# ziadabohalawa/6DoF-Pose-Estimation-and-Defect-Projection

Measured on AMD Instinct MI355X. Metric: Mrays/s ray-mesh + ICP iters/s, 640x576 vs 100k-tri mesh, higher is better.
Workload: dtype f32 rays / f64 ICP (f32 MFMA filter)

## Files before the change

6dof-pose-estimation-and-defect-projection_amd/_lib.py:

```python
import ctypes as C
import os
import sys
import threading

import numpy as np

_HERE = os.path.dirname(os.path.abspath(__file__))
LIB_PATH = os.environ.get("PEDP_LIB", os.path.join(_HERE, "libpedp_hip.so"))

HOST, DEVICE = 0, 1
POINT_TO_PLANE, POINT_TO_POINT = 0, 1


class PreprocessParams(C.Structure):
    _fields_ = [("voxel_size", C.c_double), ("plane_distance", C.c_double), ("plane_iterations", C.c_int32),
                ("first_frame", C.c_int32), ("seed", C.c_uint64), ("normal_radius", C.c_double), ("normal_max_nn", C.c_int32),
                ("cluster_min_points", C.c_int32), ("cluster_eps", C.c_double), ("outlier_neighbors", C.c_int32),
                ("flags", C.c_int32), ("outlier_std_ratio", C.c_double), ("average_normal_voxel", C.c_double)]

ALLREDUCE_FN = C.CFUNCTYPE(C.c_int, C.c_void_p, C.c_void_p, C.c_int, C.c_void_p)


class IcpParams(C.Structure):
    _fields_ = [
# ... 71 lines not shown
    "pedp_cloud_create": (C.c_int, [C.c_void_p, C.c_void_p, C.c_void_p, C.c_int64, _P(C.c_void_p)]),
    "pedp_cloud_create_device": (C.c_int, [C.c_void_p, C.c_void_p, C.c_void_p, C.c_int64, _P(C.c_void_p)]),
    "pedp_cloud_destroy": (None, [C.c_void_p]),
    "pedp_cloud_size": (C.c_int, [C.c_void_p, _P(C.c_int64), _P(C.c_int)]),
    "pedp_icp_graph_captures": (C.c_int, [C.c_void_p, _P(C.c_int64)]),
    "pedp_cloud_set_target_order": (C.c_int, [C.c_void_p, C.c_int]),
    "pedp_cloud_target_order": (C.c_int, [C.c_void_p, _P(C.c_int)]),
    "pedp_debug_target_pack": (C.c_int, [C.c_void_p, C.c_void_p, _P(C.c_int64), _P(C.c_int64), C.c_void_p, C.c_void_p,
                                         C.c_void_p, C.c_void_p, C.c_void_p]),
    "pedp_icp": (C.c_int, [C.c_void_p, C.c_void_p, C.c_void_p, _P(IcpParams), C.c_void_p, C.c_void_p,
                           _P(C.c_double), _P(C.c_double), _P(C.c_int32), C.c_void_p, C.c_void_p]),
    "pedp_icp_batched": (C.c_int, [C.c_void_p, C.c_void_p, C.c_void_p, _P(IcpParams), C.c_void_p, C.c_int,
                                   C.c_void_p, C.c_void_p, C.c_void_p]),
    "pedp_icp_batched_ex": (C.c_int, [C.c_void_p, C.c_void_p, C.c_void_p, _P(IcpParams), C.c_void_p, C.c_int,
                                      C.c_void_p, C.c_void_p, C.c_void_p, C.c_void_p]),
    "pedp_nn": (C.c_int, [C.c_void_p, C.c_void_p, C.c_void_p, C.c_void_p, C.c_void_p, C.c_void_p]),
    "pedp_nn_last_sweep_ms": (C.c_int, [C.c_void_p, _P(C.c_float)]),
    "pedp_icp_last_stats": (C.c_int, [C.c_void_p, _P(C.c_int64), _P(C.c_int64), _P(C.c_int64)]),
    "pedp_icp_last_planned_passes": (C.c_int, [C.c_void_p, _P(C.c_int64)]),
    "pedp_icp_last_serial_path": (C.c_int, [C.c_void_p, _P(C.c_int64), _P(C.c_int64)]),
    "pedp_icp_last_head_closed": (C.c_int, [C.c_void_p, _P(C.c_int64), _P(C.c_int64), _P(C.c_int64)]),
    "pedp_icp_last_certified": (C.c_int, [C.c_void_p, _P(C.c_int64), _P(C.c_int64)]),
    "pedp_icp_last_steady": (C.c_int, [C.c_void_p, _P(C.c_int64), _P(C.c_int64)]),
    "pedp_debug_nn_bf16": (C.c_int, [C.c_void_p, C.c_void_p, C.c_int64, C.c_void_p, C.c_int64, C.c_void_p]),
    "pedp_debug_icp_path": (C.c_int, [C.c_void_p, C.c_void_p, C.c_void_p]),
    "pedp_icp_begin": (C.c_int, [C.c_void_p, C.c_void_p, C.c_void_p, _P(IcpParams), C.c_void_p, C.c_int]),
    "pedp_icp_end": (C.c_int, [C.c_void_p, C.c_void_p, _P(C.c_double), _P(C.c_double), _P(C.c_int32), C.c_void_p, C.c_void_p]),
    "pedp_icp_configure": (C.c_int, [C.c_void_p, C.c_int, C.c_int]),
    "pedp_comm_unique_id": (C.c_int, [C.c_void_p]),
    "pedp_comm_create": (C.c_int, [C.c_void_p, C.c_void_p, C.c_int, C.c_int]),
    "pedp_comm_destroy": (C.c_int, [C.c_void_p]),
    "pedp_comm_size": (C.c_int, [C.c_void_p, _P(C.c_int), _P(C.c_int)]),
    "pedp_comm_allgather": (C.c_int, [C.c_void_p, C.c_void_p, C.c_void_p, C.c_int64]),
    "pedp_comm_allreduce_f64": (C.c_int, [C.c_void_p, C.c_void_p, C.c_int64]),
    "pedp_render": (C.c_int, [C.c_void_p, C.c_void_p, C.c_int64, C.c_void_p, C.c_int64, C.c_void_p, C.c_void_p, C.c_void_p,
                              C.c_void_p, C.c_int, C.c_int, C.c_void_p, C.c_void_p, C.c_int, C.c_void_p, C.c_int, C.c_void_p,
                              C.c_void_p, C.c_void_p, C.c_void_p]),
    "pedp_rasterize": (C.c_int, [C.c_void_p, C.c_void_p, C.c_int, C.c_int64, C.c_void_p, C.c_int64, C.c_int, C.c_int, C.c_int,
                                 C.c_void_p]),
    "pedp_interpolate": (C.c_int, [C.c_void_p, C.c_void_p, C.c_int, C.c_int64, C.c_int, C.c_void_p, C.c_int, C.c_int, C.c_int,
                                   C.c_void_p, C.c_int64, C.c_int, C.c_void_p]),
    "pedp_texture": (C.c_int, [C.c_void_p, C.c_void_p, C.c_int, C.c_int, C.c_int, C.c_int, C.c_void_p, C.c_int, C.c_int, C.c_int,
                               C.c_int, C.c_void_p]),
    "pedp_render_configure": (C.c_int, [C.c_void_p, C.c_int]),
    "pedp_warp_perspective": (C.c_int, [C.c_void_p, C.c_void_p, C.c_void_p, C.c_int, C.c_int, C.c_int, C.c_int, C.c_int,
                                        C.c_int, C.c_void_p]),
# ... 629 lines not shown
    a, b = C.c_int64(0), C.c_int64(0)
    check(load().pedp_icp_last_serial_path(ctx._h, C.byref(a), C.byref(b)), "pedp_icp_last_serial_path")
    return a.value, b.value


def icp_last_head_closed(ctx, rebuilds=False):
    a, b, c = C.c_int64(0), C.c_int64(0), C.c_int64(0)
    check(load().pedp_icp_last_head_closed(ctx._h, C.byref(a), C.byref(b), C.byref(c)), "pedp_icp_last_head_closed")
    return (a.value, b.value, c.value) if rebuilds else a.value


def icp_last_certified(ctx):
    a, b = C.c_int64(0), C.c_int64(0)
    check(load().pedp_icp_last_certified(ctx._h, C.byref(a), C.byref(b)), "pedp_icp_last_certified")
    return a.value, b.value


def icp_last_steady(ctx):
    a, b = C.c_int64(0), C.c_int64(0)
    check(load().pedp_icp_last_steady(ctx._h, C.byref(a), C.byref(b)), "pedp_icp_last_steady")
    return a.value, b.value


ICP_SWITCHES = ("nn_f32", "unfused_finish", "no_visit_plan", "serial_close", "copy_bracket", "head_close", "cert", "steady")
ICP_PATH_FIELDS = ("fused", "dev_result", "copy_bracket", "head", "certify", "plan", "serial_close", "unfused_finish", "exchange",
                   "steady", "steady_from")


class IcpSwitches(C.Structure):
    _fields_ = [(n, C.c_int) for n in ICP_SWITCHES + ("steady_from", "steady_grid", "target_order")]


class IcpPathInputs(C.Structure):
    _fields_ = [("n_source", C.c_int64), ("n_target", C.c_int64), ("radius", C.c_double)] + [
        (n, C.c_int) for n in ("unit_size", "poses", "timed_pass", "exhaustive", "exchange", "batch", "early_exit", "no_steady", "resident")]


class IcpPath(C.Structure):
    _fields_ = [(n, C.c_int) for n in ICP_PATH_FIELDS]


def icp_path(switches=None, steady_from=5, n_source=1, n_target=1, radius=1.0, unit_size=1, poses=1, timed_pass=-1, **flags):
    sw = None
    if switches is not None:
        sw = IcpSwitches(steady_from=int(steady_from), **{n: 1 for n in switches})
    q = IcpPathInputs(n_source=int(n_source), n_target=int(n_target), radius=float(radius), unit_size=int(unit_size), poses=int(poses),
                      timed_pass=int(timed_pass), **{n: int(bool(v)) for n, v in flags.items()})
    out = IcpPath()
    check(load().pedp_debug_icp_path(C.byref(sw) if sw is not None else None, C.byref(q), C.byref(out)), "pedp_debug_icp_path")
    return {n: (getattr(out, n) if n == "steady_from" else bool(getattr(out, n))) for n in ICP_PATH_FIELDS}


def icp_graph_captures(ctx):
# ... 205 lines not shown
```

6dof-pose-estimation-and-defect-projection_amd/csrc/icp/common.h:

```cpp
#pragma once
#include "../pedp_internal.h"
#include <cmath>
#include <cstddef>
#include <type_traits>

#ifndef PEDP_NN_EXPERIMENT
#define PEDP_NN_EXPERIMENT 0
#endif

#ifndef PEDP_ICP_STAMPS
#define PEDP_ICP_STAMPS 0
#endif
#if PEDP_ICP_STAMPS
__device__ long long g_icp_stamps[3][4096][8];
#define PEDP_STAMP(kern, unit, slot)                                                   \
    do {                                                                               \
        if ((unit) < 4096) g_icp_stamps[kern][unit][slot] = (long long)__builtin_amdgcn_s_memtime(); \
    } while (0)
extern "C" int pedp_debug_icp_stamps(long long *out) {
    return hipMemcpyFromSymbol(out, HIP_SYMBOL(g_icp_stamps), sizeof(long long) * 3 * 4096 * 8) == hipSuccess ? 0 : -3;
}
__device__ long long g_icp_rt[32][512][8];
__device__ long long g_icp_wave[512][8][16];
#define PEDP_WV(slot, val)                                                                         \
// ... 45 lines not shown
    int iters;
    int fb_count;
    int n_cand;
    int n_blocks;
    int n_segs, seg_len;
    long long sum_tiles;
    long long sum_cand;
    long long sum_fb;
    int rebuild;
    int n_rebuilds;
    int n_live;
    double r2, r2cut, r2live;
    double reachE, margin;
    double rel_fitness, rel_rmse, n_source;
    float r1, r_search, wide_radius, r2f;
    int pass, max_iter;
    double mu_theta, mu_tau;
    unsigned ticket_base, idle_base;
    int n_planned;
    int nonce;
    int n_wide;
    int n_head;
    int n_steady;
    int reserved_;
    double T_init[16];
    long long sum_cert, sum_searched;
};

constexpr double CERT_PACK = 67108864.0;
#ifndef PEDP_ICP_KAPPA
#define PEDP_ICP_KAPPA 1.25f
#endif
#ifndef PEDP_ICP_CERT_SLACK
#define PEDP_ICP_CERT_SLACK 1.0f
#endif

__device__ __forceinline__ double dmul(double a, double b) { return __dmul_rn(a, b); }
__device__ __forceinline__ double dadd(double a, double b) { return __dadd_rn(a, b); }
__device__ __forceinline__ double dsub(double a, double b) { return __dsub_rn(a, b); }

__device__ __forceinline__ double dist2(double ax, double ay, double az, double bx, double by, double bz) {
    double dx = dsub(ax, bx), dy = dsub(ay, by), dz = dsub(az, bz);
    return dadd(dadd(dmul(dx, dx), dmul(dy, dy)), dmul(dz, dz));
}

#define PEDP_GLOBAL __attribute__((address_space(1)))
template <typename T>
// ... 6 lines not shown
```

6dof-pose-estimation-and-defect-projection_amd/csrc/icp/steady_pass.h:

```cpp
#pragma once
#include "fused_pass.h"

namespace {

constexpr unsigned STEADY_SPIN_CAP = 1u << 21;
constexpr int STEADY_HANDBACK = 2;

__device__ __forceinline__ float load_sc1(const float *p) {
    return __uint_as_float(__hip_atomic_load((g_u32 *)(uintptr_t)p, __ATOMIC_RELAXED, __HIP_MEMORY_SCOPE_AGENT));
}

__global__ __launch_bounds__(BK_W * 64, 4) void icp_steady_kernel(IcpState *st0, const PassArgs a0) {
    constexpr int W = BK_W;
    static_assert(W == 8 && CH == 128, "a chunk is two halves of four 16-slot sub-blocks");
    __shared__ IcpState cur;
    typedef double __attribute__((may_alias)) state_word;
    typedef int v4i __attribute__((ext_vector_type(4)));
    constexpr int SWORDS = (int)(sizeof(IcpState) / sizeof(double));
    __shared__ PassArgs sa;
    __shared__ FinishLds<W * 64, 1> fin;
    __shared__ double wp[W][3][16], accsh[W][PSTRIDE], wfd[W][16];
    __shared__ float wcs[W][3][16], wrho[W][16], wcert[W][16];
    __shared__ int wpi[W][16], wkk[W][16], wfj[W][16], misc[4];
    __shared__ float4 wsph0[64];
    __shared__ double rP[2][3][CH], rT[3][CH], rN[3][CH];
    __shared__ float rc[CH];
    __shared__ int rj[CH], rpi[CH];
    if (threadIdx.x == 0) { sa = a0; misc[0] = 0; }
    const PassArgs &a = sa;
    const int G = (int)gridDim.x;
    const int chunk_first = a0.live_list[blockIdx.x < (unsigned)a0.n_chunks ? blockIdx.x : 0];
    v4i vis = {0, 0, 0, 0};
    if (a0.visit && blockIdx.x < (unsigned)a0.visit_cap) vis = ((const v4i *)a0.visit)[(size_t)(a0.launch & 1) * a0.visit_cap + blockIdx.x];
    for (int k = 0; k < 4; ++k) vis[k] = __builtin_amdgcn_readfirstlane(vis[k]);
    if (threadIdx.x < 64) wsph0[threadIdx.x] = a0.word_sph[(int)threadIdx.x < a0.n_words ? threadIdx.x : 0];
    bool need_close = false;
    {
        IcpState *sA = st0 + (a0.launch & 1), *sB = st0 + ((a0.launch + 1) & 1);
        double wA = 0.0, wB = 0.0;
        if (threadIdx.x < SWORDS) {
            wA = ((const state_word *)sA)[threadIdx.x];
            wB = ((const state_word *)sB)[threadIdx.x];
        }
        if (a0.launch > 0 && sB->pass == a0.launch - 1 && sB->done == 0 && sB->rebuild == 0 && sB->pass < sB->max_iter) need_close = true;
        else if (sA->pass != a0.launch || sA->done) return;
        if (threadIdx.x < SWORDS) ((state_word *)&cur)[threadIdx.x] = need_close ? wB : wA;
        __syncthreads();
    }
    auto uni = [](int v) { return __builtin_amdgcn_readfirstlane(v); };
    auto unif = [](float v) { return __int_as_float(__builtin_amdgcn_readfirstlane(__float_as_int(v))); };
    const int n_live = uni(cur.n_live), max_iter = uni(cur.max_iter);
    const unsigned base0 = (unsigned)uni((int)cur.idle_base);
    int n_part = n_live < G ? n_live : G;
    n_part = n_part < 1 ? 1 : n_part;
    g_u32 *const counters = (g_u32 *)(uintptr_t)(a0.ticket + 32);
    if ((int)blockIdx.x >= n_part) {
        if (threadIdx.x == 0) __hip_atomic_fetch_add(counters + 32 * (blockIdx.x & 15), 1u, __ATOMIC_RELAXED, __HIP_MEMORY_SCOPE_AGENT);
        return;
    }
    const bool service = (int)blockIdx.x == n_part - 1;
    const bool planned = a0.visit != nullptr && n_live <= G && vis[2] == uni(cur.nonce) + a0.launch + 1 && vis[3] == n_live;
    const double dinf = __longlong_as_double(0x7FF0000000000000ll);
    const double dnan = __longlong_as_double(0x7FF8000000000000ll);
    unsigned arrivals = 0u;
    int handovers = 0;
    auto hand_over = [&](int p_stamp) -> bool {
        (void)p_stamp;
        PEDP_RT(p_stamp, 2);
        asm volatile("s_waitcnt vmcnt(0)" ::: "memory");
        __syncthreads();
        if (threadIdx.x == 0) __hip_atomic_fetch_add(counters + 32 * (blockIdx.x & 15), 1u, __ATOMIC_RELAXED, __HIP_MEMORY_SCOPE_AGENT);
        PEDP_RT(p_stamp, 3);
        arrivals += handovers == 0 ? (unsigned)G : (unsigned)n_part;
        ++handovers;
        if (threadIdx.x < 64) {
            for (unsigned spins = 0;; ++spins) {
                unsigned c = threadIdx.x < 16 ? __hip_atomic_load(counters + 32 * threadIdx.x, __ATOMIC_RELAXED, __HIP_MEMORY_SCOPE_AGENT) : 0u;
#pragma unroll
                for (int off = 8; off >= 1; off >>= 1) c += __shfl_xor(c, off, 64);
                if (__shfl(c, 0, 64) - base0 >= arrivals) break;
                if (spins > STEADY_SPIN_CAP) {
                    if (threadIdx.x == 0) misc[0] = 1;
                    break;
                }
                __builtin_amdgcn_s_sleep(8);
            }
        }
        PEDP_RT(p_stamp, 4);
        __syncthreads();
        if (misc[0] != 0) {
            if (threadIdx.x == 0 && a0.down) *(int *)((char *)a0.down + offsetof(IcpState, done)) = -1;
            return false;
        }
        return true;
    };
    auto leave = [&](bool handback) {
        if (!service) return;
        const int tid = threadIdx.x;
        const int next = uni(cur.done) != 0 ? uni(cur.pass) + 1 : uni(cur.pass);
        if (tid < SWORDS) ((PEDP_GLOBAL state_word *)(uintptr_t)(st0 + (next & 1)))[tid] = ((const state_word *)&cur)[tid];
        if (tid == 0 && handback) as_global(&(st0 + ((next + 1) & 1))->pass)[0] = -1;
        if (!a0.down) return;
        __syncthreads();
        if (tid == 0 && handback) cur.done = STEADY_HANDBACK;
        __syncthreads();
        if (tid < SWORDS) ((state_word *)a0.down)[tid] = ((const state_word *)&cur)[tid];
    };

    bool ran = false;
    for (int p = a0.launch;; ++p) {
        if (need_close) {
            const int q = p - 1;
            FinishArgs f;
            f.live = nullptr; f.live_list = nullptr; f.n_lw = 0; f.partials = a0.partials + (size_t)(q & 1) * a0.part_stride; f.packet = nullptr; f.phase = 0;
            f.estimator = a0.estimator; f.trace = nullptr; f.hist = nullptr; f.bcx = a0.bc[0]; f.bcy = a0.bc[1]; f.bcz = a0.bc[2];
            f.serial = 0;
            f.known = 1; f.k_pass = q; f.k_rebuild = 0; f.k_n_live = n_live;
            icp_finish_body<W * 64, 1, true, 3>(&cur, f, fin, threadIdx.x);
            PEDP_RT(p, 7);
            const double pk31 = fin.pk[PACKET + 2];
            const long long searched = (long long)(pk31 / CERT_PACK);
            const long long certified = (long long)(pk31 - (double)searched * CERT_PACK);
            const bool stopped = uni(cur.done) != 0;
            const bool handback = !stopped && (uni(cur.rebuild) != 0 || (q >= a0.launch && searched * 8 > searched + certified));
            if (threadIdx.x == 0) {
                if (q >= a0.launch) cur.n_steady += 1;
                if (q >= max_iter) cur.n_head -= 1;
                cur.idle_base = base0 + arrivals;
                if (planned && !stopped && !handback) cur.n_planned += 1;
            }
            if (service) {
                const int tid = threadIdx.x;
                if (sa.trace && tid < 18)
                    as_global(sa.trace)[18 * q + tid] = tid == 0 ? cur.fitness : (tid == 1 ? cur.rmse : fin.t0[tid >= 2 ? tid - 2 : 0]);
                if (!stopped && tid < 16) as_global(sa.hist)[16 * (q + 1) + tid] = cur.upd[tid];
                if (!stopped && tid < PACKET) as_global(sa.packet)[tid] = fin.pk[tid];
            }
            __syncthreads();
            if (stopped || handback) {
                if (handovers == 0 && !hand_over(31)) return;
                if (threadIdx.x == 0) cur.idle_base = base0 + arrivals;
                __syncthreads();
                leave(handback);
                return;
            }
        } else if (uni(cur.rebuild) != 0) {
            if (!hand_over(31)) return;
            if (threadIdx.x == 0) cur.idle_base = base0 + arrivals;
            __syncthreads();
            leave(true);
            return;
        }
        need_close = true;
        PEDP_RT(p, 0);
        for (int it = 0;; ++it) {
            int tid = threadIdx.x;
            asm volatile("" : "+v"(tid));
            const int lane = tid & 63, wv = __builtin_amdgcn_readfirstlane(tid >> 6);
            const int half = wv >> 2, q4 = wv & 3;
            const int j = lane & 15, g = lane >> 4;
            const unsigned long long lt = (1ull << lane) - 1ull;
// ... 245 lines not shown
```

6dof-pose-estimation-and-defect-projection_amd/csrc/pedp_icp.hip:

```cpp
#include "pedp_internal.h"
#include <atomic>
#include <cmath>
#include <cstddef>
#include <cstdlib>
#include <cstring>
#include <new>

#if defined(__HIP_DEVICE_COMPILE__) && !defined(__gfx950__)
#error "pedp_icp.hip: the fence-free close of a pass rests on gfx950's caches; build with --offload-arch=gfx950 only"
#endif

#include "icp/common.h"
#include "icp/prep.h"
#include "icp/target_order.h"
#include "icp/segmented_sweep.h"
#include "icp/segmented_select.h"
#include "icp/solve.h"
#include "icp/ransac.h"
#include "icp/fused_close.h"
#include "icp/fused_pass.h"
#include "icp/steady_pass.h"

namespace {

// ... 5 lines not shown
    double bc[3];
};

inline size_t align_up(size_t x, size_t a) { return (x + a - 1) / a * a; }

struct IcpWorkspace {
    IcpState *st;
    double *P, *d2, *partials, *packet, *trace;
    float4 *B, *blk_sph;
    pedp_cloud_t source, target;
    const float4 *tgt4, *tile_sph;
    const int32_t *src_perm, *tgt_perm;
    float *eps, *S;
    int32_t *idx, *fb, *list;
    unsigned long long *mask;
    int32_t *blk_cnt, *blk_segstart;
    int32_t *seg_blk, *seg_rank0, *seg_n;
    float *tr_b1, *tr_b2;
    int32_t *tr_t1;
    int64_t Ns_pad, Nt_pad, blocks_cap;
    int n_words, max_segs;
    int qt;
    double *Pk, *hist, *cpart, *Tprev;
    float *cert;
    unsigned *ticket;
    unsigned long long *live;
    int32_t *live_list;
    int4 *visit;
    int2 *dur;
    int visit_cap;
    int n_lw, n_chunks;
    const float4 *word_sph;
    const double *tgt_s;
    size_t pose_stride;
};

inline int iter_capacity(int max_iter) { return (max_iter + 2 + 63) / 64 * 64; }

int carve_workspace(pedp_ctx_t c, int64_t Ns, int64_t Nt, int max_iter, int qt, IcpWorkspace &w, bool fused = false,
                    int poses = 1) {
    w = IcpWorkspace{};
    w.qt = qt;
    w.Ns_pad = (int64_t)align_up((size_t)(Ns > 0 ? Ns : 1), NN_PTS_PER_WG);
    w.Nt_pad = (int64_t)align_up((size_t)(Nt > 0 ? Nt : 1), 16 * NN_TU);
    w.blocks_cap = w.Ns_pad / (NN_SB * 16) + 1;
    const int64_t n_tiles = w.Nt_pad / (16 * qt);
// ... 33 lines not shown
    take(w.B, sizeof(float4) * (size_t)w.Ns_pad);
    take(w.eps, sizeof(float) * (size_t)w.Ns_pad);
    take(w.S, sizeof(float) * (size_t)w.Ns_pad);
    take(w.idx, sizeof(int32_t) * (size_t)w.Ns_pad);
    take(w.fb, sizeof(int32_t) * (size_t)w.Ns_pad);
    take(w.list, sizeof(int32_t) * (size_t)w.Ns_pad);
    take(w.blk_sph, sizeof(float4) * NN_SB * (size_t)w.blocks_cap);
    take(w.mask, sizeof(unsigned long long) * (size_t)w.blocks_cap * (size_t)w.n_words);
    take(w.blk_cnt, sizeof(int32_t) * (size_t)w.blocks_cap);
    take(w.blk_segstart, sizeof(int32_t) * (size_t)(w.blocks_cap + 1));
    take(w.seg_blk, sizeof(int32_t) * (size_t)w.max_segs);
    take(w.seg_rank0, sizeof(int32_t) * (size_t)w.max_segs);
    take(w.seg_n, sizeof(int32_t) * (size_t)w.max_segs);
    const size_t tr = (size_t)w.max_segs * 4 * (NN_SB * 16);
    take(w.tr_b1, sizeof(float) * tr);
    take(w.tr_t1, sizeof(int32_t) * tr);
    take(w.tr_b2, sizeof(float) * tr);
    if (fused) {
        take(w.Pk, sizeof(double) * 3 * (size_t)w.Ns_pad * 2);
        take(w.Tprev, sizeof(double) * 3 * (size_t)w.Ns_pad * 2);
        take(w.cert, sizeof(float) * (size_t)w.Ns_pad * (poses <= 1 ? 2 : 0));
        take(w.hist, sizeof(double) * 16 * (size_t)iter_capacity(max_iter));
        take(w.cpart, sizeof(double) * PSTRIDE * (size_t)w.blocks_cap * 2);
        take(w.ticket, 17 * 128);
        take(w.live, sizeof(unsigned long long) * 2 * (size_t)w.n_lw);
        take(w.live_list, sizeof(int32_t) * (size_t)w.blocks_cap);
        if (poses <= 1) {
            w.visit_cap = (int)(w.blocks_cap < 2 * c->num_cus ? w.blocks_cap : 2 * c->num_cus);
            take(w.visit, (sizeof(int4) + sizeof(int2)) * 2 * (size_t)w.visit_cap);
        }
    }
    PEDP_REQUIRE(n_slots <= MAX_SLOTS, "pedp_icp: carve_workspace lays out %d buffers, its table holds %d", n_slots, MAX_SLOTS);
    off = align_up(off, 4096);
    w.pose_stride = off;
    int st = c->icp_ws.reserve(off * (size_t)(poses > 0 ? poses : 1));
    if (st) return st;
    for (int k = 0; k < n_slots; ++k) {
        char *buf = (char *)c->icp_ws.ptr + slot[k].off;
        memcpy((char *)&w + slot[k].member, &buf, sizeof(buf));
    }
    if (w.visit) w.dur = (int2 *)(w.visit + 2 * (size_t)w.visit_cap);
    if (!fused) PEDP_HIP_CHECK(hipMemsetAsync(w.blk_cnt, 0, sizeof(int32_t) * (size_t)w.blocks_cap, c->stream));
    return PEDP_OK;
}

inline size_t zeroed_span_bytes(const IcpWorkspace &w) {
// ... 25 lines not shown
    double r2cut;
};
inline IcpRadii icp_radii(double r, double r_cull) {
    IcpRadii k;
    k.r1 = (float)(r * 1.01);
    k.r_search = (float)(r_cull * (1.0 + 1e-6)) + 1e-6f;
    k.r2f = (float)(r * r) * 1.00001f;
    k.r2cut = r_cull * r_cull * (1.0 + 1e-12);
    return k;
}

using IcpSwitches = pedp_icp_switches;
inline const IcpSwitches &icp_switches() {
    static const IcpSwitches sw = [] {
        auto flag = [](const char *name, int unset) { const char *v = getenv(name); return v ? atoi(v) != 0 : unset; };
        auto num = [](const char *name, int unset) { const char *v = getenv(name); return v && *v ? atoi(v) : unset; };
        const char *order = getenv("PEDP_ICP_TARGET_ORDER");
        IcpSwitches s;
        s.nn_f32 = flag("PEDP_NN_F32", 0); s.unfused_finish = flag("PEDP_ICP_UNFUSED_FINISH", 0);
        s.no_visit_plan = flag("PEDP_ICP_NO_VISIT_PLAN", 0); s.serial_close = flag("PEDP_ICP_SERIAL_CLOSE", 0);
        s.copy_bracket = flag("PEDP_ICP_COPY_BRACKET", 0); s.head_close = flag("PEDP_ICP_HEAD_CLOSE", 1);
        s.cert = flag("PEDP_ICP_CERT", 1); s.steady = flag("PEDP_ICP_STEADY", 1);
        s.steady_from = num("PEDP_ICP_STEADY_FROM", 5); s.steady_grid = num("PEDP_ICP_STEADY_GRID", 0);
        s.target_order = order && !strcmp(order, "hilbert") ? PEDP_TARGET_ORDER_HILBERT
                         : order && !strcmp(order, "compact") ? PEDP_TARGET_ORDER_COMPACT : PEDP_TARGET_ORDER_AUTO;
        return s;
    }();
    return sw;
}

using IcpPath = pedp_icp_path;
using IcpPathInputs = pedp_icp_path_inputs;
inline bool fused_eligible(int qt, bool exhaustive, double r, int64_t Ns, int64_t Nt) {
    return qt == 1 && !exhaustive && r > 0.0 && Ns > 0 && Nt > 0 && (Nt + 1023) / 1024 <= BK_WCAP;
}
inline IcpPath icp_decide_path(const IcpSwitches &sw, const IcpPathInputs &in) {
    IcpPath p{};
    p.fused = fused_eligible(in.unit_size, in.exhaustive, in.radius, in.n_source, in.n_target);
    p.copy_bracket = sw.copy_bracket; p.exchange = in.exchange;
    p.steady_from = sw.steady_from < 1 ? 1 : sw.steady_from;
    if (!p.fused) return p;
    const bool single = in.poses <= 1;
    const bool closes_itself = !in.exchange && !sw.unfused_finish;
    p.serial_close = sw.serial_close; p.unfused_finish = sw.unfused_finish;
    p.plan = single && !sw.no_visit_plan;
    p.certify = single && closes_itself && sw.cert;
// ... 111 lines not shown
    pa.fuse = !path.exchange && !path.unfused_finish ? 1 : 0;
    pa.n_lw = w.n_lw; pa.packet = w.packet; pa.trace = job.want_trace ? w.trace : nullptr; pa.ticket = w.ticket;
    pa.down = path.dev_result ? (unsigned long long *)((char *)x->pinned + RESULT_OFF) : nullptr;
    pa.serial_close = path.serial_close; pa.head = path.head; pa.launch = 0;
    pa.part_stride = (size_t)PSTRIDE * (size_t)w.blocks_cap;
    pa.cert = path.certify ? w.cert : nullptr; pa.cert_stride = (size_t)w.Ns_pad;
    pa.visit = path.plan ? w.visit : nullptr; pa.dur = path.plan ? w.dur : nullptr; pa.visit_cap = w.visit_cap; pa.n_cu = x->num_cus;
}

struct PassLaunch {
    int pass = 0;
    bool steady_launch = false;
    hipEvent_t ev0 = nullptr, ev1 = nullptr;
};

int enqueue_fused_pass(pedp_ctx_t c, const IcpJob &job, const PassLaunch &l) {
    PassArgs pa = job.pa;
    pa.launch = pa.head ? l.pass : 0;
    int64_t g = job.w.n_chunks;
    if (g > 2 * c->num_cus) g = 2 * c->num_cus;
    if (g < 1) g = 1;
    if (pa.head) g += 1;
    if (l.ev0) PEDP_HIP_CHECK(hipEventRecord(l.ev0, c->stream));
    if (l.steady_launch)
        hipLaunchKernelGGL(icp_steady_kernel, dim3((unsigned)steady_grid(c)), dim3(BK_W * 64), 0, c->stream, job.w.st, pa);
    else if (job.in.poses > 1)
        hipLaunchKernelGGL((icp_pass_kernel<BK_W, true>), dim3((unsigned)g, (unsigned)job.in.poses), dim3(BK_W * 64), 0, c->stream, job.w.st, pa);
    else
        hipLaunchKernelGGL((icp_pass_kernel<BK_W, false>), dim3((unsigned)g), dim3(BK_W * 64), 0, c->stream, job.w.st, pa);
    if (l.ev1) { PEDP_HIP_CHECK(hipEventRecord(l.ev1, c->stream)); c->nn_timed = true; }
    PEDP_HIP_CHECK(hipGetLastError());
    return PEDP_OK;
}

void launch_finish(pedp_ctx_t x, const IcpJob &job, int stage) {
    const IcpWorkspace &w = job.w;
    hipLaunchKernelGGL(icp_finish_kernel, dim3((unsigned)job.in.poses), dim3(FIN_THREADS), 0, x->stream, w.st, w.live, w.live_list, w.n_lw,
                       w.cpart, w.packet, stage, job.estimator, job.pa.trace, w.hist, job.tp.bc[0], job.tp.bc[1], job.tp.bc[2],
                       job.pa.pose_stride, job.pa.serial_close);
}

int ensure_spatial_perm(pedp_ctx_t c, pedp_cloud_t cl) {
    if (cl->N == 0 || cl->perm) return PEDP_OK;
    const int64_t n_chunks = (cl->N + 127) / 128;
    size_t perm_cap = 0, sph_cap = 0;
    void *perm = c->cloud_pool.take(sizeof(int32_t) * (size_t)cl->N, &perm_cap);
    void *sph = c->cloud_pool.take(sizeof(double) * 32 * (size_t)n_chunks, &sph_cap);
    auto fail = [&](int rc, const char *what) {
// ... 403 lines not shown
        copies = true;
    }
    if (copies || !job.steady_held) PEDP_HIP_CHECK(hipStreamSynchronize(x->stream));
    const IcpState *hp = (const IcpState *)((const char *)x->pinned + (job.path.dev_result ? RESULT_OFF : 0));
    if (job.path.dev_result && hp->done == 0) {
        pedp_set_error("pedp_icp: the registration's final state did not arrive");
        return PEDP_ERR_HIP;
    }
    if (hp->done < 0) {
        pedp_set_error("pedp_icp: a pass could not be closed (workgroups of its launch did not sign off in time)");
        return PEDP_ERR_HIP;
    }
    for (int k = 0; k < 16; ++k) T_out[k] = hp->T[k];
    x->icp_last_cand = job.path.fused ? hp->sum_tiles * 256 : hp->sum_tiles * (16 * job.in.unit_size) * (NN_SB * 16);
    x->icp_last_fb = hp->sum_fb;
    x->icp_last_passes = hp->iters + 1;
    x->icp_last_planned = hp->n_planned;
    x->icp_last_wide = hp->n_wide;
    x->icp_last_head = hp->n_head;
    x->icp_last_cert = hp->sum_cert;
    x->icp_last_searched = hp->sum_searched;
    x->icp_last_steady = hp->n_steady;
    x->icp_last_handbacks = handbacks;
    x->icp_last_rebuilds = hp->n_rebuilds;
    x->icp_last_bracket = (job.path.copy_bracket ? 0 : 1) + (job.path.dev_result ? 2 : 0);
    x->icp_last_nt = job.in.n_target;
    if (fitness) *fitness = hp->fitness;
    if (inlier_rmse) *inlier_rmse = hp->rmse;
    if (n_iter_done) *n_iter_done = hp->iters;
    return PEDP_OK;
}

bool graph_key_equal(const pedp_icp_graph_key &a, const pedp_icp_graph_key &b) {
    return a.src_gen == b.src_gen && a.tgt_gen == b.tgt_gen && a.ws == b.ws && a.Ns == b.Ns && a.Nt == b.Nt &&
           a.max_iter == b.max_iter && a.qt == b.qt && a.estimator == b.estimator && a.r == b.r &&
           a.rel_fitness == b.rel_fitness && a.rel_rmse == b.rel_rmse && a.seg == b.seg && a.poses == b.poses;
}

template <typename Enqueue>
int capture_graph(pedp_ctx_t x, hipGraphExec_t &exec, hipError_t &e, Enqueue enqueue) {
    if (exec) { (void)hipGraphExecDestroy(exec); exec = nullptr; }
    e = hipStreamBeginCapture(x->stream, hipStreamCaptureModeThreadLocal);
    if (e != hipSuccess) return PEDP_OK;
    hipGraph_t graph = nullptr;
    const int rc = enqueue();
    e = hipStreamEndCapture(x->stream, &graph);
// ... 455 lines not shown
}

int pedp_icp_last_serial_path(pedp_ctx_t c, int64_t *wide_closes, int64_t *bracket) {
    PEDP_REQUIRE(c && wide_closes && bracket, "pedp_icp_last_serial_path: null argument");
    *wide_closes = c->icp_last_wide;
    *bracket = c->icp_last_bracket;
    return PEDP_OK;
}

int pedp_icp_last_certified(pedp_ctx_t c, int64_t *slots, int64_t *searched_slots) {
    PEDP_REQUIRE(c && slots, "pedp_icp_last_certified: null argument");
    *slots = c->icp_last_cert;
    if (searched_slots) *searched_slots = c->icp_last_searched;
    return PEDP_OK;
}

int pedp_icp_last_steady(pedp_ctx_t c, int64_t *passes, int64_t *handbacks) {
    PEDP_REQUIRE(c && passes, "pedp_icp_last_steady: null argument");
    *passes = c->icp_last_steady;
    if (handbacks) *handbacks = c->icp_last_handbacks;
    return PEDP_OK;
}

int pedp_icp_last_head_closed(pedp_ctx_t c, int64_t *head_closed, int64_t *rebuilds, int64_t *launches) {
    PEDP_REQUIRE(c && head_closed, "pedp_icp_last_head_closed: null argument");
    *head_closed = c->icp_last_head;
    if (rebuilds) *rebuilds = c->icp_last_rebuilds;
    if (launches) *launches = c->icp_last_launches;
    return PEDP_OK;
}

int pedp_nn_last_sweep_ms(pedp_ctx_t c, float *ms) {
    PEDP_REQUIRE(c && ms, "pedp_nn_last_sweep_ms: null argument");
    PEDP_REQUIRE(c->nn_timed, "pedp_nn_last_sweep_ms: no timed sweep has run on this context");
    PEDP_HIP_CHECK(hipSetDevice(c->device));
    if (c->nn_pairs > 0) {
        float sum = 0.f;
        for (int k = 0; k < c->nn_pairs; ++k) {
            float one = 0.f;
            PEDP_HIP_CHECK(hipEventSynchronize(c->nn_evs[2 * k + 1]));
            PEDP_HIP_CHECK(hipEventElapsedTime(&one, c->nn_evs[2 * k], c->nn_evs[2 * k + 1]));
            sum += one;
        }
        *ms = sum / (float)c->nn_pairs;
        return PEDP_OK;
    }
// ... 8 lines not shown
```

6dof-pose-estimation-and-defect-projection_amd/csrc/pedp_internal.h:

```cpp
#pragma once
#include <hip/hip_runtime.h>
#include <cstdarg>
#include <cstdint>
#include <cstdio>
#include <cstring>
#include <mutex>
#include <vector>
#include "../../include/pedp.h"

void pedp_set_error(const char *fmt, ...);
uint64_t pedp_next_generation();
struct pedp_ctx_s;
int pedp_upload(pedp_ctx_s *c, void *dst, const void *src, size_t bytes);
int pedp_download(pedp_ctx_s *c, void *dst, const void *src, size_t bytes);
int pedp_download_view(pedp_ctx_s *c, const void *src, size_t bytes, const void **view);
int pedp_download_parts(pedp_ctx_s *c, const void *src, size_t span, int n, const size_t *off, void *const *dst, const size_t *bytes);
struct pedp_ctx_s;
int pedp_sort_keys64_begin(pedp_ctx_s *c, int64_t N, int bits, unsigned long long **d_keys);
int pedp_sort_keys64_run(pedp_ctx_s *c, int64_t N, int bits, int32_t *d_perm);
int pedp_sort_keys64_exact_begin(pedp_ctx_s *c, int64_t N, int bits, unsigned long long **d_keys);
int pedp_sort_keys64_exact_run(pedp_ctx_s *c, int64_t N, int bits, int32_t *d_perm);

__host__ __device__ inline bool pedp_row_finite(const double *pts, int64_t i) {
    uint64_t b[3];
// ... 81 lines not shown
    int nn_pairs = 0;
    int nn_span_launches = 1;
    pedp_scratch icp_ws;
    pedp_scratch ops;
    pedp_scratch sort_ws;
    pedp_pool cloud_pool;
    pedp_scratch ops_small;
    pedp_scratch chain;
    void *avg_host = nullptr;
    size_t avg_host_cap = 0;
    pedp_scratch ops_in;
    pedp_scratch proj, proj_out;
    pedp_scratch render_ws;
    pedp_scratch render_io;
    pedp_scratch crop_ws;
    pedp_scratch crop_io;
    pedp_scratch pose_ws;
    pedp_scratch pose_io;
    pedp_scratch stats_ws;
    pedp_scratch stats_io;
    int render_chunk = 0;
    bool icp_exhaustive = false;
    int icp_timed_pass = -1;
    long long icp_last_cand = 0, icp_last_fb = 0, icp_last_passes = 0, icp_last_nt = 0, icp_last_planned = 0, icp_last_wide = 0, icp_last_bracket = 0, icp_last_head = 0, icp_last_rebuilds = 0, icp_last_launches = 0, icp_last_cert = 0, icp_last_searched = 0, icp_last_steady = 0, icp_last_handbacks = 0;
    void *icp_pending = nullptr;
    pedp_ctx_s *sub[PEDP_MAX_SUB] = {};
    hipGraphExec_t icp_graph = nullptr;
    pedp_icp_graph_key icp_graph_key;
    hipGraphExec_t icp_bgraph[18] = {};
    pedp_icp_graph_key icp_bgraph_key[18];
    long long icp_graph_captures = 0;
    void *pinned = nullptr;
    size_t pinned_cap = 0;
    void *stage[2] = {nullptr, nullptr};
    size_t stage_cap[2] = {0, 0};
    bool stage_busy = false;
    pedp_scratch metrics_ws;
    pedp_scratch metrics_io;
    pedp_scratch closest_ws;
    pedp_scratch closest_io;
    int closest_mode = 0;
};

#define PEDP_TRI_STRIDE 12

struct pedp_mesh_s {
    pedp_ctx_t ctx = nullptr;
// ... 51 lines not shown
```

include/pedp.h:

```cpp
#ifndef PEDP_H
#define PEDP_H
#include <stdint.h>
#ifdef __cplusplus
extern "C" {
#endif

typedef enum {
    PEDP_OK = 0,
    PEDP_ERR_BAD_ARG = -1,
    PEDP_ERR_NO_NORMALS = -2,
    PEDP_ERR_HIP = -3,
    PEDP_ERR_ALLOC = -4,
    PEDP_ERR_COLLECTIVE = -5
} pedp_status;

enum { PEDP_HOST = 0, PEDP_DEVICE = 1 };
enum { PEDP_POINT_TO_PLANE = 0, PEDP_POINT_TO_POINT = 1 };

typedef struct pedp_ctx_s *pedp_ctx_t;
typedef struct pedp_mesh_s *pedp_mesh_t;
typedef struct pedp_rayset_s *pedp_rayset_t;
typedef struct pedp_cloud_s *pedp_cloud_t;

int pedp_version(void);
// ... 169 lines not shown
            int32_t *idx, double *d2);
int pedp_nn_last_sweep_ms(pedp_ctx_t ctx, float *ms);

int pedp_ransac_hypotheses(pedp_ctx_t ctx, pedp_cloud_t source, pedp_cloud_t target, const int32_t *corr, uint64_t seed,
                           int64_t itr0, int count, double edge_similarity, double max_distance, double normal_angle,
                           uint8_t *accepted, double *T);

int pedp_icp_configure(pedp_ctx_t ctx, int exhaustive, int timed_pass);

int pedp_icp_last_stats(pedp_ctx_t ctx, int64_t *passes, int64_t *pairs_swept, int64_t *fallback_points);

int pedp_icp_last_planned_passes(pedp_ctx_t ctx, int64_t *planned);

int pedp_icp_graph_captures(pedp_ctx_t ctx, int64_t *captures);

int pedp_icp_last_serial_path(pedp_ctx_t ctx, int64_t *wide_closes, int64_t *bracket);

int pedp_icp_last_head_closed(pedp_ctx_t ctx, int64_t *head_closed, int64_t *rebuilds, int64_t *launches);

int pedp_icp_last_certified(pedp_ctx_t ctx, int64_t *slots, int64_t *searched_slots);

int pedp_icp_last_steady(pedp_ctx_t ctx, int64_t *passes, int64_t *handbacks);

int pedp_debug_nn_bf16(pedp_ctx_t ctx, const float *src4, int64_t n_src, const float *tgt4, int64_t n_tgt, float *g);

int pedp_debug_target_pack(pedp_ctx_t ctx, pedp_cloud_t cloud, int64_t *rows, int64_t *pad_rows, int32_t *tile_perm,
                           float *tgt4, float *sph16, float *sph64, float *sph1024);

typedef struct pedp_icp_switches {
    int nn_f32, unfused_finish, no_visit_plan, serial_close, copy_bracket;
    int head_close, cert, steady;
    int steady_from;
    int steady_grid;
    int target_order;
} pedp_icp_switches;
typedef struct pedp_icp_path_inputs {
    int64_t n_source, n_target;
    double radius;
    int unit_size;
    int poses;
    int timed_pass;
    int exhaustive;
    int exchange;
    int batch;
    int early_exit;
    int no_steady;
    int resident;
} pedp_icp_path_inputs;
typedef struct pedp_icp_path {
    int fused;
    int dev_result;
    int copy_bracket;
    int head;
    int certify, plan;
    int serial_close;
    int unfused_finish;
    int exchange;
// ... 229 lines not shown
```

Before: 690.5.

## Let steady-kernel followers copy closed ICP state instead of redundantly closing

In the persistent steady ICP kernel, every block used to run the full finish/close reduction each pass. Now only the first C blocks (defaulting to the CU count) act as closers. Each closer publishes its resulting state plus certification word into a tagged per-pass record, and the remaining blocks spin on that tag and copy the state. This removes redundant finish work on the extra blocks at the cost of cross-block spin-waiting and extra global stores. A spin cap flags failure, and a counter of followers is exposed.

```diff
diff --git a/6dof-pose-estimation-and-defect-projection_amd/_lib.py b/6dof-pose-estimation-and-defect-projection_amd/_lib.py
--- a/6dof-pose-estimation-and-defect-projection_amd/_lib.py
+++ b/6dof-pose-estimation-and-defect-projection_amd/_lib.py
@@ -117,6 +117,7 @@
     "pedp_icp_last_head_closed": (C.c_int, [C.c_void_p, _P(C.c_int64), _P(C.c_int64), _P(C.c_int64)]),
     "pedp_icp_last_certified": (C.c_int, [C.c_void_p, _P(C.c_int64), _P(C.c_int64)]),
     "pedp_icp_last_steady": (C.c_int, [C.c_void_p, _P(C.c_int64), _P(C.c_int64)]),
+    "pedp_icp_last_steady_followers": (C.c_int, [C.c_void_p, _P(C.c_int64)]),
     "pedp_debug_nn_bf16": (C.c_int, [C.c_void_p, C.c_void_p, C.c_int64, C.c_void_p, C.c_int64, C.c_void_p]),
     "pedp_debug_icp_path": (C.c_int, [C.c_void_p, C.c_void_p, C.c_void_p]),
     "pedp_icp_begin": (C.c_int, [C.c_void_p, C.c_void_p, C.c_void_p, _P(IcpParams), C.c_void_p, C.c_int]),
@@ -792,13 +793,19 @@
     return a.value, b.value
 
 
+def icp_last_steady_followers(ctx):
+    a = C.c_int64(0)
+    check(load().pedp_icp_last_steady_followers(ctx._h, C.byref(a)), "pedp_icp_last_steady_followers")
+    return a.value
+
+
 ICP_SWITCHES = ("nn_f32", "unfused_finish", "no_visit_plan", "serial_close", "copy_bracket", "head_close", "cert", "steady")
 ICP_PATH_FIELDS = ("fused", "dev_result", "copy_bracket", "head", "certify", "plan", "serial_close", "unfused_finish", "exchange",
                    "steady", "steady_from")
 
 
 class IcpSwitches(C.Structure):
-    _fields_ = [(n, C.c_int) for n in ICP_SWITCHES + ("steady_from", "steady_grid", "target_order")]
+    _fields_ = [(n, C.c_int) for n in ICP_SWITCHES + ("steady_from", "steady_grid", "target_order", "steady_closers")]
 
 
 class IcpPathInputs(C.Structure):
diff --git a/6dof-pose-estimation-and-defect-projection_amd/csrc/icp/common.h b/6dof-pose-estimation-and-defect-projection_amd/csrc/icp/common.h
--- a/6dof-pose-estimation-and-defect-projection_amd/csrc/icp/common.h
+++ b/6dof-pose-estimation-and-defect-projection_amd/csrc/icp/common.h
@@ -91,7 +91,7 @@
     int n_wide;
     int n_head;
     int n_steady;
-    int reserved_;
+    int n_followed;
     double T_init[16];
     long long sum_cert, sum_searched;
 };
diff --git a/6dof-pose-estimation-and-defect-projection_amd/csrc/icp/steady_pass.h b/6dof-pose-estimation-and-defect-projection_amd/csrc/icp/steady_pass.h
--- a/6dof-pose-estimation-and-defect-projection_amd/csrc/icp/steady_pass.h
+++ b/6dof-pose-estimation-and-defect-projection_amd/csrc/icp/steady_pass.h
@@ -5,12 +5,40 @@
 
 constexpr unsigned STEADY_SPIN_CAP = 1u << 21;
 constexpr int STEADY_HANDBACK = 2;
+constexpr int FOLLOW_STRIDE = 128;
+constexpr int FOLLOW_TAG = 112;
+static_assert(sizeof(IcpState) / sizeof(double) + 1 <= FOLLOW_TAG, "the record ends in front of the tag's line");
 
 __device__ __forceinline__ float load_sc1(const float *p) {
     return __uint_as_float(__hip_atomic_load((g_u32 *)(uintptr_t)p, __ATOMIC_RELAXED, __HIP_MEMORY_SCOPE_AGENT));
 }
 
-__global__ __launch_bounds__(BK_W * 64, 4) void icp_steady_kernel(IcpState *st0, const PassArgs a0) {
+__device__ __forceinline__ bool steady_follow(IcpState *cur, double *word, int *failed, const double *rec, unsigned tag) {
+    constexpr int SWORDS = (int)(sizeof(IcpState) / sizeof(double));
+    typedef double __attribute__((may_alias)) state_word;
+    if (threadIdx.x < 64) {
+        for (unsigned spins = 0;; ++spins) {
+            const unsigned t = (unsigned)__builtin_amdgcn_readfirstlane((int)__hip_atomic_load((g_u32 *)(uintptr_t)(rec + FOLLOW_TAG), __ATOMIC_RELAXED, __HIP_MEMORY_SCOPE_AGENT));
+            if (t == tag) break;
+            if (spins > STEADY_SPIN_CAP) {
+                if (threadIdx.x == 0) *failed = 1;
+                break;
+            }
+            __builtin_amdgcn_s_sleep(2);
+        }
+    }
+    __syncthreads();
+    if (*failed != 0) return false;
+    if (threadIdx.x <= SWORDS) {
+        const double v = load_sc1(&rec[threadIdx.x]);
+        if (threadIdx.x < SWORDS) ((state_word *)cur)[threadIdx.x] = v;
+        else *word = v;
+    }
+    __syncthreads();
+    return true;
+}
+
+__global__ __launch_bounds__(BK_W * 64, 4) void icp_steady_kernel(IcpState *st0, const PassArgs a0, double *follow, int follow_cap, int closers) {
     constexpr int W = BK_W;
     static_assert(W == 8 && CH == 128, "a chunk is two halves of four 16-slot sub-blocks");
     __shared__ IcpState cur;
@@ -23,6 +51,7 @@
     __shared__ float wcs[W][3][16], wrho[W][16], wcert[W][16];
     __shared__ int wpi[W][16], wkk[W][16], wfj[W][16], misc[4];
     __shared__ float4 wsph0[64];
+    __shared__ double *role_rec[2];
     __shared__ double rP[2][3][CH], rT[3][CH], rN[3][CH];
     __shared__ float rc[CH];
     __shared__ int rj[CH], rpi[CH];
@@ -58,7 +87,21 @@
         if (threadIdx.x == 0) __hip_atomic_fetch_add(counters + 32 * (blockIdx.x & 15), 1u, __ATOMIC_RELAXED, __HIP_MEMORY_SCOPE_AGENT);
         return;
     }
-    const bool service = (int)blockIdx.x == n_part - 1;
+    bool service;
+    {
+        int C = follow != nullptr && closers >= 1 && closers < n_part ? closers : n_part;
+        C = C > follow_cap ? n_part : C;
+        const bool closer = (int)blockIdx.x < C;
+        const bool publishes = closer && (int)blockIdx.x + C < n_part;
+        service = (int)blockIdx.x == C - 1;
+        if (threadIdx.x == 0) {
+            misc[1] = (closer ? 1 : 0) | (publishes ? 2 : 0);
+            misc[2] = n_part - C;
+            for (int k = 0; k < 2; ++k)
+                role_rec[k] = C < n_part ? follow + ((size_t)k * follow_cap + (size_t)((int)blockIdx.x % C)) * FOLLOW_STRIDE : nullptr;
+        }
+        __syncthreads();
+    }
     const bool planned = a0.visit != nullptr && n_live <= G && vis[2] == uni(cur.nonce) + a0.launch + 1 && vis[3] == n_live;
     const double dinf = __longlong_as_double(0x7FF0000000000000ll);
     const double dnan = __longlong_as_double(0x7FF8000000000000ll);
@@ -97,6 +140,8 @@
     auto leave = [&](bool handback) {
         if (!service) return;
         const int tid = threadIdx.x;
+        if (tid == 0) cur.n_followed = misc[2];
+        __syncthreads();
         const int next = uni(cur.done) != 0 ? uni(cur.pass) + 1 : uni(cur.pass);
         if (tid < SWORDS) ((PEDP_GLOBAL state_word *)(uintptr_t)(st0 + (next & 1)))[tid] = ((const state_word *)&cur)[tid];
         if (tid == 0 && handback) as_global(&(st0 + ((next + 1) & 1))->pass)[0] = -1;
@@ -111,19 +156,25 @@
     for (int p = a0.launch;; ++p) {
         if (need_close) {
             const int q = p - 1;
-            FinishArgs f;
-            f.live = nullptr; f.live_list = nullptr; f.n_lw = 0; f.partials = a0.partials + (size_t)(q & 1) * a0.part_stride; f.packet = nullptr; f.phase = 0;
-            f.estimator = a0.estimator; f.trace = nullptr; f.hist = nullptr; f.bcx = a0.bc[0]; f.bcy = a0.bc[1]; f.bcz = a0.bc[2];
-            f.serial = 0;
-            f.known = 1; f.k_pass = q; f.k_rebuild = 0; f.k_n_live = n_live;
-            icp_finish_body<W * 64, 1, true, 3>(&cur, f, fin, threadIdx.x);
+            const bool closer = (uni(misc[1]) & 1) != 0;
+            if (closer) {
+                FinishArgs f;
+                f.live = nullptr; f.live_list = nullptr; f.n_lw = 0; f.partials = a0.partials + (size_t)(q & 1) * a0.part_stride; f.packet = nullptr; f.phase = 0;
+                f.estimator = a0.estimator; f.trace = nullptr; f.hist = nullptr; f.bcx = a0.bc[0]; f.bcy = a0.bc[1]; f.bcz = a0.bc[2];
+                f.serial = 0;
+                f.known = 1; f.k_pass = q; f.k_rebuild = 0; f.k_n_live = n_live;
+                icp_finish_body<W * 64, 1, true, 3>(&cur, f, fin, threadIdx.x);
+            } else if (!steady_follow(&cur, &fin.pk[PACKET + 2], &misc[0], role_rec[q & 1], (unsigned)(uni(cur.nonce) + q + 1))) {
+                if (threadIdx.x == 0 && a0.down) *(int *)((char *)a0.down + offsetof(IcpState, done)) = -1;
+                return;
+            }
             PEDP_RT(p, 7);
             const double pk31 = fin.pk[PACKET + 2];
             const long long searched = (long long)(pk31 / CERT_PACK);
             const long long certified = (long long)(pk31 - (double)searched * CERT_PACK);
             const bool stopped = uni(cur.done) != 0;
             const bool handback = !stopped && (uni(cur.rebuild) != 0 || (q >= a0.launch && searched * 8 > searched + certified));
-            if (threadIdx.x == 0) {
+            if (closer && threadIdx.x == 0) {
                 if (q >= a0.launch) cur.n_steady += 1;
                 if (q >= max_iter) cur.n_head -= 1;
                 cur.idle_base = base0 + arrivals;
@@ -137,6 +188,13 @@
                 if (!stopped && tid < PACKET) as_global(sa.packet)[tid] = fin.pk[tid];
             }
             __syncthreads();
+            if ((uni(misc[1]) & 2) != 0 && threadIdx.x < 64) {
+                double *const rec = role_rec[q & 1];
+                const unsigned tag = (unsigned)(uni(cur.nonce) + q + 1);
+                for (int k = threadIdx.x; k <= SWORDS; k += 64) store_sc1(&rec[k], k < SWORDS ? ((const state_word *)&cur)[k] : pk31);
+                asm volatile("s_waitcnt vmcnt(0)" ::: "memory");
+                if (threadIdx.x == 0) __hip_atomic_store((g_u32 *)(uintptr_t)(rec + FOLLOW_TAG), tag, __ATOMIC_RELAXED, __HIP_MEMORY_SCOPE_AGENT);
+            }
             if (stopped || handback) {
                 if (handovers == 0 && !hand_over(31)) return;
                 if (threadIdx.x == 0) cur.idle_base = base0 + arrivals;
diff --git a/6dof-pose-estimation-and-defect-projection_amd/csrc/pedp_icp.hip b/6dof-pose-estimation-and-defect-projection_amd/csrc/pedp_icp.hip
--- a/6dof-pose-estimation-and-defect-projection_amd/csrc/pedp_icp.hip
+++ b/6dof-pose-estimation-and-defect-projection_amd/csrc/pedp_icp.hip
@@ -51,6 +51,8 @@
     int n_words, max_segs;
     int qt;
     double *Pk, *hist, *cpart, *Tprev;
+    double *follow;
+    int follow_cap;
     float *cert;
     unsigned *ticket;
     unsigned long long *live;
@@ -130,6 +132,8 @@
         take(w.cert, sizeof(float) * (size_t)w.Ns_pad * (poses <= 1 ? 2 : 0));
         take(w.hist, sizeof(double) * 16 * (size_t)iter_capacity(max_iter));
         take(w.cpart, sizeof(double) * PSTRIDE * (size_t)w.blocks_cap * 2);
+        w.follow_cap = poses <= 1 ? (int)(w.blocks_cap < 2 * c->num_cus ? w.blocks_cap : 2 * c->num_cus) : 0;
+        take(w.follow, sizeof(double) * FOLLOW_STRIDE * 2 * (size_t)w.follow_cap);
         take(w.ticket, 17 * 128);
         take(w.live, sizeof(unsigned long long) * 2 * (size_t)w.n_lw);
         take(w.live_list, sizeof(int32_t) * (size_t)w.blocks_cap);
@@ -201,6 +205,7 @@
         s.copy_bracket = flag("PEDP_ICP_COPY_BRACKET", 0); s.head_close = flag("PEDP_ICP_HEAD_CLOSE", 1);
         s.cert = flag("PEDP_ICP_CERT", 1); s.steady = flag("PEDP_ICP_STEADY", 1);
         s.steady_from = num("PEDP_ICP_STEADY_FROM", 5); s.steady_grid = num("PEDP_ICP_STEADY_GRID", 0);
+        s.steady_closers = num("PEDP_ICP_STEADY_CLOSERS", 0);
         s.target_order = order && !strcmp(order, "hilbert") ? PEDP_TARGET_ORDER_HILBERT
                          : order && !strcmp(order, "compact") ? PEDP_TARGET_ORDER_COMPACT : PEDP_TARGET_ORDER_AUTO;
         return s;
@@ -358,8 +363,11 @@
     if (g < 1) g = 1;
     if (pa.head) g += 1;
     if (l.ev0) PEDP_HIP_CHECK(hipEventRecord(l.ev0, c->stream));
-    if (l.steady_launch)
-        hipLaunchKernelGGL(icp_steady_kernel, dim3((unsigned)steady_grid(c)), dim3(BK_W * 64), 0, c->stream, job.w.st, pa);
+    if (l.steady_launch) {
+        const int asked = icp_switches().steady_closers;
+        hipLaunchKernelGGL(icp_steady_kernel, dim3((unsigned)steady_grid(c)), dim3(BK_W * 64), 0, c->stream, job.w.st, pa,
+                           job.w.follow_cap > 0 ? job.w.follow : nullptr, job.w.follow_cap, asked > 0 ? asked : c->num_cus);
+    }
     else if (job.in.poses > 1)
         hipLaunchKernelGGL((icp_pass_kernel<BK_W, true>), dim3((unsigned)g, (unsigned)job.in.poses), dim3(BK_W * 64), 0, c->stream, job.w.st, pa);
     else
@@ -809,6 +817,7 @@
     x->icp_last_searched = hp->sum_searched;
     x->icp_last_steady = hp->n_steady;
     x->icp_last_handbacks = handbacks;
+    x->icp_last_followed = hp->n_followed;
     x->icp_last_rebuilds = hp->n_rebuilds;
     x->icp_last_bracket = (job.path.copy_bracket ? 0 : 1) + (job.path.dev_result ? 2 : 0);
     x->icp_last_nt = job.in.n_target;
@@ -1310,6 +1319,12 @@
     return PEDP_OK;
 }
 
+int pedp_icp_last_steady_followers(pedp_ctx_t c, int64_t *followers) {
+    PEDP_REQUIRE(c && followers, "pedp_icp_last_steady_followers: null argument");
+    *followers = c->icp_last_followed;
+    return PEDP_OK;
+}
+
 int pedp_icp_last_head_closed(pedp_ctx_t c, int64_t *head_closed, int64_t *rebuilds, int64_t *launches) {
     PEDP_REQUIRE(c && head_closed, "pedp_icp_last_head_closed: null argument");
     *head_closed = c->icp_last_head;
diff --git a/6dof-pose-estimation-and-defect-projection_amd/csrc/pedp_internal.h b/6dof-pose-estimation-and-defect-projection_amd/csrc/pedp_internal.h
--- a/6dof-pose-estimation-and-defect-projection_amd/csrc/pedp_internal.h
+++ b/6dof-pose-estimation-and-defect-projection_amd/csrc/pedp_internal.h
@@ -127,7 +127,7 @@
     int render_chunk = 0;
     bool icp_exhaustive = false;
     int icp_timed_pass = -1;
-    long long icp_last_cand = 0, icp_last_fb = 0, icp_last_passes = 0, icp_last_nt = 0, icp_last_planned = 0, icp_last_wide = 0, icp_last_bracket = 0, icp_last_head = 0, icp_last_rebuilds = 0, icp_last_launches = 0, icp_last_cert = 0, icp_last_searched = 0, icp_last_steady = 0, icp_last_handbacks = 0;
+    long long icp_last_cand = 0, icp_last_fb = 0, icp_last_passes = 0, icp_last_nt = 0, icp_last_planned = 0, icp_last_wide = 0, icp_last_bracket = 0, icp_last_head = 0, icp_last_rebuilds = 0, icp_last_launches = 0, icp_last_cert = 0, icp_last_searched = 0, icp_last_steady = 0, icp_last_handbacks = 0, icp_last_followed = 0;
     void *icp_pending = nullptr;
     pedp_ctx_s *sub[PEDP_MAX_SUB] = {};
     hipGraphExec_t icp_graph = nullptr;
diff --git a/include/pedp.h b/include/pedp.h
--- a/include/pedp.h
+++ b/include/pedp.h
@@ -215,6 +215,8 @@
 
 int pedp_icp_last_steady(pedp_ctx_t ctx, int64_t *passes, int64_t *handbacks);
 
+int pedp_icp_last_steady_followers(pedp_ctx_t ctx, int64_t *followers);
+
 int pedp_debug_nn_bf16(pedp_ctx_t ctx, const float *src4, int64_t n_src, const float *tgt4, int64_t n_tgt, float *g);
 
 int pedp_debug_target_pack(pedp_ctx_t ctx, pedp_cloud_t cloud, int64_t *rows, int64_t *pad_rows, int32_t *tile_perm,
@@ -226,6 +228,7 @@
     int steady_from;
     int steady_grid;
     int target_order;
+    int steady_closers;
 } pedp_icp_switches;
 typedef struct pedp_icp_path_inputs {
     int64_t n_source, n_target;
```

After: 719.1 (median of 6 runs). +4.2%, better.
